# megvii-research/basedet

Measured on AMD Instinct MI355X. Metric: images/sec training RetinaNet-R50-FPN 1333x800, higher is better.
Workload: dtype bf16; 1 GPU; retinanet_r50_800x1344 train step (fwd+bwd+allreduce+SGD), DummyLoader boxes, random-init weights, inputs resident in HBM; per_gpu_batch=16, global_batch=16, parallelism=dp1

## Files before the change

### basedet_amd/csrc/gskip.hip

```cpp
#include "common.h"

namespace {

enum { GS_ANY = 1, GS_TOP = 2, GS_BOT = 4, GS_LEFT = 8, GS_RIGHT = 16, GS_TL = 32, GS_TR = 64, GS_BL = 128, GS_BR = 256 };

struct GsSeg { int patch_start, H, W, pw, off; };

struct GsParams {
    const bf16_raw* g;
    int* mask;
    int C, ppi, ph, pw_px, nseg, patches_per_img, total;
    GsSeg seg[BD_MAX_SEGS];
};

__device__ __forceinline__ int gs_level(const GsParams& p, int rem) {
    int s = 0;
#pragma unroll
    for (int k = 1; k < BD_MAX_SEGS; ++k)
        if (k < p.nseg && rem >= p.seg[k].patch_start) s = k;
    return s;
}

__global__ __launch_bounds__(256) void gskip_scan_kernel(const GsParams p) {
    __shared__ int sbits;
    const int tid = threadIdx.x;
    const int pid = blockIdx.x;
    const int n = pid / p.patches_per_img, rem = pid - n * p.patches_per_img;
    const int s = gs_level(p, rem);
    const int H = p.seg[s].H, W = p.seg[s].W, pwn = p.seg[s].pw;
    const int local = rem - p.seg[s].patch_start, by = local / pwn, bx = local - by * pwn;
    const int y0 = by * p.ph, x0 = bx * p.pw_px;
    const int cpp = p.C >> 3;
    const int items = p.ph * p.pw_px * cpp;
    const long long img = (long long)n * p.ppi + p.seg[s].off;
    if (tid == 0) sbits = 0;
    __syncthreads();
    int bits = 0;
    constexpr int U = 8;
    for (int b = 0; b < items; b += 256 * U) {
        u32x4_t v[U];
        int pix[U];
#pragma unroll
        for (int k = 0; k < U; ++k) {
            const int i = b + k * 256 + tid;
            v[k] = (u32x4_t){0u, 0u, 0u, 0u};
            pix[k] = -1;
            if (i < items) {
                const int px = i / cpp, ch = i - px * cpp;
                const int py = px / p.pw_px, pxx = px - py * p.pw_px;
                const int y = y0 + py, x = x0 + pxx;
                if (y < H && x < W) {
                    v[k] = *reinterpret_cast<const u32x4_t*>(p.g + (img + (long long)y * W + x) * p.C + ch * 8);
                    pix[k] = px;
                }
            }
        }
#pragma unroll
        for (int k = 0; k < U; ++k) {
            if (pix[k] >= 0 && (v[k][0] | v[k][1] | v[k][2] | v[k][3])) {
                const int py = pix[k] / p.pw_px, pxx = pix[k] - py * p.pw_px;
                const bool t = py == 0, bo = py == p.ph - 1, l = pxx == 0, r = pxx == p.pw_px - 1;
                bits |= GS_ANY | (t ? GS_TOP : 0) | (bo ? GS_BOT : 0) | (l ? GS_LEFT : 0) | (r ? GS_RIGHT : 0) | (t && l ? GS_TL : 0) |
                        (t && r ? GS_TR : 0) | (bo && l ? GS_BL : 0) | (bo && r ? GS_BR : 0);
            }
        }
    }
#pragma unroll
    for (int m = 32; m >= 1; m >>= 1) bits |= __shfl_xor(bits, m, 64);
    if ((tid & 63) == 0 && bits) atomicOr(&sbits, bits);
    __syncthreads();
    if (tid == 0) p.mask[pid] = sbits;
}

template <bool FRESH>
__device__ __forceinline__ int gs_mask(const int* m, int i) {
    if (FRESH) return __hip_atomic_load(m + i, __ATOMIC_RELAXED, __HIP_MEMORY_SCOPE_AGENT);
    return m[i];
}

template <bool FRESH>
__device__ __forceinline__ void gs_compact_body(const GsParams& p, int* live, int* list, int* count, int* wsum) {
    constexpr int KP = 8;
    const int tid = threadIdx.x, wv = tid >> 6, ln = tid & 63;
    int base = 0;
    for (int c0 = 0; c0 < p.total; c0 += 1024 * KP) {
        int lv[KP];
#pragma unroll
        for (int j = 0; j < KP; ++j) {
            const int q = c0 + tid * KP + j;
            lv[j] = 0;
            if (q < p.total) {
                const int n = q / p.patches_per_img, rem = q - n * p.patches_per_img;
                const int s = gs_level(p, rem);
                const int pwn = p.seg[s].pw, rows = (p.seg[s].H + p.ph - 1) / p.ph;
                const int local = rem - p.seg[s].patch_start, by = local / pwn, bx = local - by * pwn;
                const int* m = p.mask + (long long)n * p.patches_per_img + p.seg[s].patch_start;
                const bool up = by > 0, dn = by + 1 < rows, lf = bx > 0, rt = bx + 1 < pwn;
                int v = gs_mask<FRESH>(m, by * pwn + bx) & GS_ANY;
                if (up) v |= gs_mask<FRESH>(m, (by - 1) * pwn + bx) & GS_BOT;
                if (dn) v |= gs_mask<FRESH>(m, (by + 1) * pwn + bx) & GS_TOP;
                if (lf) v |= gs_mask<FRESH>(m, by * pwn + bx - 1) & GS_RIGHT;
                if (rt) v |= gs_mask<FRESH>(m, by * pwn + bx + 1) & GS_LEFT;
                if (up && lf) v |= gs_mask<FRESH>(m, (by - 1) * pwn + bx - 1) & GS_BR;
                if (up && rt) v |= gs_mask<FRESH>(m, (by - 1) * pwn + bx + 1) & GS_BL;
                if (dn && lf) v |= gs_mask<FRESH>(m, (by + 1) * pwn + bx - 1) & GS_TR;
                if (dn && rt) v |= gs_mask<FRESH>(m, (by + 1) * pwn + bx + 1) & GS_TL;
                lv[j] = v != 0;
            }
        }
        int cnt = 0;
#pragma unroll
        for (int j = 0; j < KP; ++j) cnt += lv[j];
        int inc = cnt;
#pragma unroll
        for (int o = 1; o < 64; o <<= 1) {
            const int y = __shfl_up(inc, o, 64);
            if (ln >= o) inc += y;
        }
        if (ln == 63) wsum[wv] = inc;
        __syncthreads();
        int off = base + inc - cnt, tot = 0;
#pragma unroll
        for (int w = 0; w < 16; ++w) {
            off += w < wv ? wsum[w] : 0;
            tot += wsum[w];
        }
#pragma unroll
        for (int j = 0; j < KP; ++j) {
            const int q = c0 + tid * KP + j;
            if (q < p.total) live[q] = lv[j];
            if (lv[j]) list[off++] = q;
        }
        base += tot;
        __syncthreads();
    }
    if (tid == 0) *count = base;
}

__global__ __launch_bounds__(1024) void gskip_compact_kernel(const GsParams p, int* live, int* list, int* count) {
    __shared__ int wsum[16];
    gs_compact_body<false>(p, live, list, count, wsum);
}

enum { GM_HDR = 8 };

struct GmSeg { int H, W, off, s4, s8, ss; };

struct GmParams {
    const bf16_raw* t;
    const int* live_in;
    int* map;
    int C, ppi, nseg, pi4, pi8, pis, tot4, tot8;
    GmSeg seg[BD_MAX_SEGS];
};

__global__ __launch_bounds__(1024) void gskip_fill_kernel(const GmParams p, const GsParams cp, int total) {
    __shared__ int sbits, slast;
    __shared__ int wsum[16];
    const int tid = threadIdx.x;
    int* m4 = p.map + GM_HDR;
    int* m8 = m4 + p.tot4;
    const int cpp = p.C >> 3;
    const int items = 4 * 16 * cpp;
    for (int pid = blockIdx.x; pid < total; pid += gridDim.x) {
        const int n = pid / p.pis, rem = pid - n * p.pis;
        int s = 0;
#pragma unroll
        for (int k = 1; k < BD_MAX_SEGS; ++k)
            if (k < p.nseg && rem >= p.seg[k].ss) s = k;
        const int H = p.seg[s].H, W = p.seg[s].W;
        const int sc = (W + 15) >> 4, r4 = (H + 3) >> 2, c8 = (W + 7) >> 3;
        const int local = rem - p.seg[s].ss, sy = local / sc, sx = local - sy * sc;
        int q4[2], q8[2];
        bool ok4[2], ok8[2], lv[2];
#pragma unroll
        for (int h = 0; h < 2; ++h) {
            ok4[h] = 2 * sy + h < r4;
            q4[h] = n * p.pi4 + p.seg[s].s4 + (2 * sy + h) * sc + sx;
            ok8[h] = 2 * sx + h < c8;
            q8[h] = n * p.pi8 + p.seg[s].s8 + sy * c8 + 2 * sx + h;
            lv[h] = ok4[h] && (p.live_in == nullptr || p.live_in[q4[h]] != 0);
        }
        int b = 0;
        if (lv[0] || lv[1]) {
            if (tid == 0) sbits = 0;
            __syncthreads();
            const long long img = (long long)n * p.ppi + p.seg[s].off;
            int bits = 0;
#pragma unroll
            for (int h = 0; h < 2; ++h) {
                if (!lv[h]) continue;
                for (int i = tid; i < items; i += 1024) {
                    const int px = i / cpp, ch = i - px * cpp;
                    const int py = px >> 4, pxx = px & 15;
                    const int y = 8 * sy + 4 * h + py, x = 16 * sx + pxx;
                    if (y < H && x < W) {
                        const u32x4_t v = *reinterpret_cast<const u32x4_t*>(p.t + (img + (long long)y * W + x) * p.C + ch * 8);
                        if (v[0] | v[1] | v[2] | v[3]) {
                            const bool t = py == 0, bo = py == 3, l = pxx == 0, r = pxx == 15;
                            const int w = GS_ANY | (t ? GS_TOP : 0) | (bo ? GS_BOT : 0) | (l ? GS_LEFT : 0) | (r ? GS_RIGHT : 0) |
                                          (t && l ? GS_TL : 0) | (t && r ? GS_TR : 0) | (bo && l ? GS_BL : 0) | (bo && r ? GS_BR : 0);
                            bits |= (w << (9 * h)) | (1 << (18 + (pxx >> 3)));
                        }
                    }
                }
            }
#pragma unroll
            for (int m = 32; m >= 1; m >>= 1) bits |= __shfl_xor(bits, m, 64);
            if ((tid & 63) == 0 && bits) atomicOr(&sbits, bits);
            __syncthreads();
            b = sbits;
            __syncthreads();
        }
        if (tid == 0) {
            if (ok4[0]) m4[q4[0]] = b & 511;
            if (ok4[1]) m4[q4[1]] = (b >> 9) & 511;
            if (ok8[0]) m8[q8[0]] = (b >> 18) & 1;
            if (ok8[1]) m8[q8[1]] = (b >> 19) & 1;
        }
    }
    if (tid == 0) {
        __builtin_amdgcn_fence(__ATOMIC_RELEASE, "agent");
        slast = atomicAdd(p.map + 1, 1) == (int)gridDim.x - 1;
    }
    __syncthreads();
    if (!slast) return;
    __builtin_amdgcn_fence(__ATOMIC_ACQUIRE, "agent");
    const int nxt = (p.map[0] & 1) ^ 1;
    int* live = m8 + p.tot8;
    gs_compact_body<true>(cp, live, live + p.tot4 * (1 + nxt), p.map + 2 + nxt, wsum);
    if (tid == 0) { p.map[0] = nxt; p.map[1] = 0; }
}

enum { FL_HDR = 8, FL_MAX_DEPTH = 8 };

struct FlSeg { int H, W, off, s4, pw; };

struct FlParams {
    const int* labels;
    int* map[FL_MAX_DEPTH];
    int A, ppi, nseg, depths, pi4, tot4;
    FlSeg seg[BD_MAX_SEGS];
};

__global__ __launch_bounds__(1024) void fwd_live_kernel(const FlParams p) {
    extern __shared__ __attribute__((aligned(16))) unsigned char fl_bm[];
    __shared__ int slast;
    __shared__ int wsum[16];
    const int tid = threadIdx.x;
    const int n = blockIdx.x / p.nseg, s = blockIdx.x - n * p.nseg;
    const int H = p.seg[s].H, W = p.seg[s].W, HW = H * W, pwn = p.seg[s].pw;
    const int npatch = ((H + 3) >> 2) * pwn;
    unsigned char* cur = fl_bm;
    unsigned char* nxt = fl_bm + HW;
    for (int i = tid; i < HW; i += 1024) cur[i] = 0;
    __syncthreads();
    const int* lab = p.labels + ((long long)n * p.ppi + p.seg[s].off) * p.A;
    for (int i = tid; i < HW * p.A; i += 1024)
        if (lab[i] > 0) cur[i / p.A] = 1;
    __syncthreads();
    for (int k = 0; k < p.depths; ++k) {
        for (int i = tid; i < HW; i += 1024) {
            const int y = i / W, x = i - y * W;
            const int y0 = y > 0 ? y - 1 : 0, y1 = y + 1 < H ? y + 1 : H - 1, x0 = x > 0 ? x - 1 : 0, x1 = x + 1 < W ? x + 1 : W - 1;
            int v = 0;
            for (int yy = y0; yy <= y1; ++yy)
                for (int xx = x0; xx <= x1; ++xx) v |= cur[yy * W + xx];
            nxt[i] = (unsigned char)v;
        }
        __syncthreads();
        int* live = p.map[k] + FL_HDR + n * p.pi4 + p.seg[s].s4;
        for (int q = tid; q < npatch; q += 1024) {
            const int by = q / pwn, bx = q - by * pwn;
            const int ye = by * 4 + 4 < H ? by * 4 + 4 : H, xe = bx * 16 + 16 < W ? bx * 16 + 16 : W;
            int v = 0;
            for (int y = by * 4; y < ye; ++y)
                for (int x = bx * 16; x < xe; ++x) v |= nxt[y * W + x];
            live[q] = v;
        }
        unsigned char* t = cur; cur = nxt; nxt = t;
        __syncthreads();
    }
    __builtin_amdgcn_fence(__ATOMIC_RELEASE, "agent");
    __syncthreads();
    if (tid == 0) slast = atomicAdd(p.map[0] + 1, 1) == (int)gridDim.x - 1;
    __syncthreads();
    if (!slast) return;
    __builtin_amdgcn_fence(__ATOMIC_ACQUIRE, "agent");
    constexpr int KP = 8;
    const int wv = tid >> 6, ln = tid & 63;
    for (int k = 0; k < p.depths; ++k) {
        int* hdr = p.map[k];
        const int* live = hdr + FL_HDR;
        const int to = (hdr[0] & 1) ^ 1;
        int* list = hdr + FL_HDR + p.tot4 * (1 + to);
        int base = 0;
        for (int c0 = 0; c0 < p.tot4; c0 += 1024 * KP) {
            int lv[KP];
            int cnt = 0;
#pragma unroll
            for (int j = 0; j < KP; ++j) {
                const int q = c0 + tid * KP + j;
                lv[j] = q < p.tot4 ? (__hip_atomic_load(live + q, __ATOMIC_RELAXED, __HIP_MEMORY_SCOPE_AGENT) != 0) : 0;
                cnt += lv[j];
            }
            int inc = cnt;
#pragma unroll
            for (int o = 1; o < 64; o <<= 1) {
                const int y = __shfl_up(inc, o, 64);
                if (ln >= o) inc += y;
            }
            if (ln == 63) wsum[wv] = inc;
            __syncthreads();
            int off = base + inc - cnt, tot = 0;
#pragma unroll
            for (int w = 0; w < 16; ++w) {
                off += w < wv ? wsum[w] : 0;
                tot += wsum[w];
            }
#pragma unroll
            for (int j = 0; j < KP; ++j)
                if (lv[j]) list[off++] = c0 + tid * KP + j;
            base += tot;
            __syncthreads();
        }
        if (tid == 0) { hdr[2 + to] = base; hdr[0] = to; }
    }
    if (tid == 0) p.map[0][1] = 0;
}

GsParams gs_params(const bd_conv_desc* d, int ph, int pw, int side = 0) {
    GsParams p{};
    p.C = side ? d->Cin : d->Cout; p.ppi = side ? d->in_pix_per_img : d->out_pix_per_img; p.ph = ph; p.pw_px = pw; p.nseg = d->nseg;
    int ps = 0;
    for (int s = 0; s < d->nseg; ++s) {
        GsSeg& sg = p.seg[s];
        const int H = side ? d->Hi[s] : d->Ho[s], W = side ? d->Wi[s] : d->Wo[s];
        sg.patch_start = ps; sg.H = H; sg.W = W; sg.pw = cdiv(W, pw); sg.off = side ? d->in_off[s] : d->out_off[s];
        ps += cdiv(H, ph) * sg.pw;
    }
    p.patches_per_img = ps;
    p.total = ps * d->N;
    return p;
}

}

int bd_gskip_patches(const bd_conv_desc* d, int ph, int pw) {
    return gs_params(d, ph, pw).total;
}

void bd_gskip_scan(const bd_conv_desc* d, const void* g, int ph, int pw, int* mask, hipStream_t stream) {
    GsParams p = gs_params(d, ph, pw);
    p.g = (const bf16_raw*)g; p.mask = mask;
    if (p.total > 0) hipLaunchKernelGGL(gskip_scan_kernel, dim3(p.total), dim3(256), 0, stream, p);
}

void bd_gskip_compact(const bd_conv_desc* d, int ph, int pw, const int* mask, int* live, int* list, int* count, hipStream_t stream) {
    GsParams p = gs_params(d, ph, pw);
    p.mask = const_cast<int*>(mask);
    hipLaunchKernelGGL(gskip_compact_kernel, dim3(1), dim3(1024), 0, stream, p, live, list, count);
}

void bd_gskip_map_layout(const bd_conv_desc* d, int side, BdGskipMap* out) {
    const int p4 = gs_params(d, 4, 16, side).total, p8 = gs_params(d, 8, 8, side).total;
    out->p4 = p4; out->p8 = p8;
    out->m4 = GM_HDR; out->m8 = GM_HDR + p4; out->live = out->m8 + p8; out->list = out->live + p4;
    out->ints = (size_t)GM_HDR + (size_t)4 * p4 + p8;
}

extern "C" size_t bd_conv2d_gskip_map_bytes(const bd_conv_desc* d, int of_dx) {
    if (!d || d->nseg < 1 || d->nseg > BD_MAX_SEGS || !(d->R == 3 && d->S == 3 && d->stride == 1 && d->pad == 1)) return 0;
    BdGskipMap m;
    bd_gskip_map_layout(d, of_dx ? 1 : 0, &m);
    return m.ints * sizeof(int);
}

void bd_gskip_fill(const bd_conv_desc* d, int side, const void* t, const int* live_in, int* map, hipStream_t stream) {
    const GsParams g4 = gs_params(d, 4, 16, side), g8 = gs_params(d, 8, 8, side), gs = gs_params(d, 8, 16, side);
    GmParams p{};
    p.t = (const bf16_raw*)t; p.live_in = live_in; p.map = map;
    p.C = g4.C; p.ppi = g4.ppi; p.nseg = g4.nseg;
    p.pi4 = g4.patches_per_img; p.pi8 = g8.patches_per_img; p.pis = gs.patches_per_img; p.tot4 = g4.total; p.tot8 = g8.total;
    for (int s = 0; s < g4.nseg; ++s)
        p.seg[s] = GmSeg{g4.seg[s].H, g4.seg[s].W, g4.seg[s].off, g4.seg[s].patch_start, g8.seg[s].patch_start, gs.seg[s].patch_start};
    GsParams cp = g4;
    cp.mask = map + GM_HDR;
    const int grid = gs.total < 128 ? gs.total : 128;
    if (grid > 0) hipLaunchKernelGGL(gskip_fill_kernel, dim3(grid), dim3(1024), 0, stream, p, cp, gs.total);
}

extern "C" int bd_gskip_map_scan(const bd_conv_desc* d, int of_dx, const void* t, void* map, size_t map_bytes, bd_stream_t stream) {
    BD_REQUIRE(d && t && map, "gskip_map_scan: null pointer");
    const size_t need = bd_conv2d_gskip_map_bytes(d, of_dx);
    BD_REQUIRE(need > 0, "gskip_map_scan: liveness maps belong to 3x3 / stride 1 / pad 1 descriptors");
    BD_REQUIRE(map_bytes >= need, "gskip_map_scan: map %zu < required %zu bytes", map_bytes, need);
    const int side = of_dx ? 1 : 0;
    BdGskipMap m;
    bd_gskip_map_layout(d, side, &m);
    int* mp = (int*)map;
    if (hipMemsetAsync(mp, 0, GM_HDR * sizeof(int), (hipStream_t)stream) != hipSuccess) { bd_set_error("gskip_map_scan: memset failed"); return BD_ELAUNCH; }
    GsParams p4 = gs_params(d, 4, 16, side), p8 = gs_params(d, 8, 8, side);
    p4.g = p8.g = (const bf16_raw*)t;
    p4.mask = mp + m.m4; p8.mask = mp + m.m8;
    if (p4.total > 0) {
        hipLaunchKernelGGL(gskip_scan_kernel, dim3(p4.total), dim3(256), 0, (hipStream_t)stream, p4);
        hipLaunchKernelGGL(gskip_scan_kernel, dim3(p8.total), dim3(256), 0, (hipStream_t)stream, p8);
    }
    hipLaunchKernelGGL(gskip_compact_kernel, dim3(1), dim3(1024), 0, (hipStream_t)stream, p4, mp + m.live, mp + m.list, mp + 2);
    BD_CHECK_LAUNCH("bd_gskip_map_scan");
    return BD_OK;
}

void bd_fwd_map_layout(const bd_conv_desc* d, BdFwdMap* out) {
    const int p4 = gs_params(d, 4, 16, 0).total;
    out->p4 = p4; out->live = FL_HDR; out->list = FL_HDR + p4;
    out->ints = (size_t)FL_HDR + (size_t)3 * p4;
}

extern "C" size_t bd_fwd_live_map_bytes(const bd_conv_desc* d) {
    if (!d || d->nseg < 1 || d->nseg > BD_MAX_SEGS || !(d->R == 3 && d->S == 3 && d->stride == 1 && d->pad == 1)) return 0;
    BdFwdMap m;
    bd_fwd_map_layout(d, &m);
    return m.ints * sizeof(int);
}

extern "C" int bd_fwd_live_maps(const bd_conv_desc* d, const int32_t* labels, int A, int depths, void* const* maps, size_t map_bytes,
                                int reset, bd_stream_t stream) {
    BD_REQUIRE(d && labels && maps, "fwd_live_maps: null pointer");
    const size_t need = bd_fwd_live_map_bytes(d);
    BD_REQUIRE(need > 0, "fwd_live_maps: forward liveness maps belong to 3x3 / stride 1 / pad 1 descriptors");
    BD_REQUIRE(A >= 1 && depths >= 1 && depths <= FL_MAX_DEPTH, "fwd_live_maps: A=%d depths=%d (1 .. %d)", A, depths, (int)FL_MAX_DEPTH);
    BD_REQUIRE(map_bytes >= need, "fwd_live_maps: map %zu < required %zu bytes", map_bytes, need);
    const GsParams g4 = gs_params(d, 4, 16, 0);
    FlParams p{};
    p.labels = labels; p.A = A; p.ppi = g4.ppi; p.nseg = g4.nseg; p.depths = depths; p.pi4 = g4.patches_per_img; p.tot4 = g4.total;
    size_t lds = 0;
    for (int s = 0; s < g4.nseg; ++s) {
        BD_REQUIRE(d->Hi[s] == d->Ho[s] && d->Wi[s] == d->Wo[s], "fwd_live_maps: level %d changes size", s);
        p.seg[s] = FlSeg{g4.seg[s].H, g4.seg[s].W, g4.seg[s].off, g4.seg[s].patch_start, g4.seg[s].pw};
        const size_t b = (size_t)2 * g4.seg[s].H * g4.seg[s].W;
        BD_REQUIRE((long long)g4.seg[s].H * g4.seg[s].W * A < 0x7fffffffll, "fwd_live_maps: level %d too large", s);
        lds = b > lds ? b : lds;
    }
    BD_REQUIRE(lds <= 160 * 1024 - 256, "fwd_live_maps: a level of %zu pixels does not fit the LDS bitmap", lds / 2);
    for (int k = 0; k < depths; ++k) {
        BD_REQUIRE(maps[k], "fwd_live_maps: null map %d", k);
        p.map[k] = (int*)maps[k];
        if (reset && hipMemsetAsync(maps[k], 0, FL_HDR * sizeof(int), (hipStream_t)stream) != hipSuccess) {
            bd_set_error("fwd_live_maps: memset failed");
            return BD_ELAUNCH;
        }
    }
    if (d->N < 1 || g4.total < 1) return BD_OK;
    BD_ONCE_PER_DEVICE((void)hipFuncSetAttribute(reinterpret_cast<const void*>(&fwd_live_kernel), hipFuncAttributeMaxDynamicSharedMemorySize,
                                                 160 * 1024 - 256));
    hipLaunchKernelGGL(fwd_live_kernel, dim3(d->N * g4.nseg), dim3(1024), lds, (hipStream_t)stream, p);
    BD_CHECK_LAUNCH("bd_fwd_live_maps");
    return BD_OK;
}
```

Baseline: 727.4 images/sec.

## Scan gradient-skip patches per wave and pack forward liveness into bitmaps

Adds a wave-per-patch scan kernel, used when patches are small, that covers four patches per wave and replaces integer division with a float-reciprocal division. The fill kernel now gives one fill patch to each wave instead of the whole 1024-thread block, gathers the mask writes in LDS and removes per-patch block barriers. The forward liveness kernel moves from a byte-per-pixel LDS map to a 32-pixel-per-word bitmap, with vectorised label loads and word-level 3x3 dilation. The aim is to cut launch, barrier and LDS costs in these auxiliary sparsity kernels, in exchange for more code paths and atomicOr contention while marking labels.

```diff
diff --git a/basedet_amd/csrc/gskip.hip b/basedet_amd/csrc/gskip.hip
--- a/basedet_amd/csrc/gskip.hip
+++ b/basedet_amd/csrc/gskip.hip
@@ -19,6 +19,25 @@
     for (int k = 1; k < BD_MAX_SEGS; ++k)
         if (k < p.nseg && rem >= p.seg[k].patch_start) s = k;
     return s;
+}
+
+__device__ __forceinline__ int gs_border_bits(int py, int pxx, int ph, int pw) {
+    const bool t = py == 0, bo = py == ph - 1, l = pxx == 0, r = pxx == pw - 1;
+    return GS_ANY | (t ? GS_TOP : 0) | (bo ? GS_BOT : 0) | (l ? GS_LEFT : 0) | (r ? GS_RIGHT : 0) | (t && l ? GS_TL : 0) |
+           (t && r ? GS_TR : 0) | (bo && l ? GS_BL : 0) | (bo && r ? GS_BR : 0);
+}
+
+__device__ __forceinline__ int gs_div(int i, int d, float inv) {
+    int q = (int)((float)i * inv);
+    q -= q * d > i;
+    q += (q + 1) * d <= i;
+    return q;
+}
+
+__device__ __forceinline__ int gs_wave_or(int bits) {
+#pragma unroll
+    for (int m = 32; m >= 1; m >>= 1) bits |= __shfl_xor(bits, m, 64);
+    return bits;
 }
 
 __global__ __launch_bounds__(256) void gskip_scan_kernel(const GsParams p) {
@@ -59,17 +78,64 @@
         for (int k = 0; k < U; ++k) {
             if (pix[k] >= 0 && (v[k][0] | v[k][1] | v[k][2] | v[k][3])) {
                 const int py = pix[k] / p.pw_px, pxx = pix[k] - py * p.pw_px;
-                const bool t = py == 0, bo = py == p.ph - 1, l = pxx == 0, r = pxx == p.pw_px - 1;
-                bits |= GS_ANY | (t ? GS_TOP : 0) | (bo ? GS_BOT : 0) | (l ? GS_LEFT : 0) | (r ? GS_RIGHT : 0) | (t && l ? GS_TL : 0) |
-                        (t && r ? GS_TR : 0) | (bo && l ? GS_BL : 0) | (bo && r ? GS_BR : 0);
-            }
-        }
-    }
-#pragma unroll
-    for (int m = 32; m >= 1; m >>= 1) bits |= __shfl_xor(bits, m, 64);
+                bits |= gs_border_bits(py, pxx, p.ph, p.pw_px);
+            }
+        }
+    }
+    bits = gs_wave_or(bits);
     if ((tid & 63) == 0 && bits) atomicOr(&sbits, bits);
     __syncthreads();
     if (tid == 0) p.mask[pid] = sbits;
+}
+
+enum { GS_WAVE_PATCHES = 4 };
+
+__global__ __launch_bounds__(256) void gskip_scan_wave_kernel(const GsParams p) {
+    const int ln = threadIdx.x & 63;
+    const int first = __builtin_amdgcn_readfirstlane((blockIdx.x * 4 + (threadIdx.x >> 6)) * GS_WAVE_PATCHES);
+    const int cpp = p.C >> 3;
+    const int items = p.ph * p.pw_px * cpp;
+    const float inv_cpp = 1.0f / (float)cpp, inv_pw = 1.0f / (float)p.pw_px;
+    constexpr int U = 8;
+    for (int j = 0; j < GS_WAVE_PATCHES; ++j) {
+        const int pid = first + j;
+        if (pid >= p.total) break;
+        const int n = pid / p.patches_per_img, rem = pid - n * p.patches_per_img;
+        const int s = gs_level(p, rem);
+        const int H = p.seg[s].H, W = p.seg[s].W, pwn = p.seg[s].pw;
+        const int local = rem - p.seg[s].patch_start, by = local / pwn, bx = local - by * pwn;
+        const int y0 = by * p.ph, x0 = bx * p.pw_px;
+        const long long img = (long long)n * p.ppi + p.seg[s].off;
+        int bits = 0;
+        for (int b = 0; b < items; b += 64 * U) {
+            u32x4_t v[U];
+            int pix[U];
+#pragma unroll
+            for (int k = 0; k < U; ++k) {
+                const int i = b + k * 64 + ln;
+                v[k] = (u32x4_t){0u, 0u, 0u, 0u};
+                pix[k] = -1;
+                if (i < items) {
+                    const int px = gs_div(i, cpp, inv_cpp), ch = i - px * cpp;
+                    const int py = gs_div(px, p.pw_px, inv_pw), pxx = px - py * p.pw_px;
+                    const int y = y0 + py, x = x0 + pxx;
+                    if (y < H && x < W) {
+                        v[k] = *reinterpret_cast<const u32x4_t*>(p.g + (img + (long long)y * W + x) * p.C + ch * 8);
+                        pix[k] = px;
+                    }
+                }
+            }
+#pragma unroll
+            for (int k = 0; k < U; ++k) {
+                if (pix[k] >= 0 && (v[k][0] | v[k][1] | v[k][2] | v[k][3])) {
+                    const int py = gs_div(pix[k], p.pw_px, inv_pw), pxx = pix[k] - py * p.pw_px;
+                    bits |= gs_border_bits(py, pxx, p.ph, p.pw_px);
+                }
+            }
+        }
+        bits = gs_wave_or(bits);
+        if (ln == 0) p.mask[pid] = bits;
+    }
 }
 
 template <bool FRESH>
@@ -142,7 +208,7 @@
     gs_compact_body<false>(p, live, list, count, wsum);
 }
 
-enum { GM_HDR = 8 };
+enum { GM_HDR = 8, GM_WAVES = 16 };
 
 struct GmSeg { int H, W, off, s4, s8, ss; };
 
@@ -155,76 +221,81 @@
 };
 
 __global__ __launch_bounds__(1024) void gskip_fill_kernel(const GmParams p, const GsParams cp, int total) {
-    __shared__ int sbits, slast;
+    __shared__ int slast;
+    __shared__ int sidx[GM_WAVES * 4], sval[GM_WAVES * 4];
     __shared__ int wsum[16];
-    const int tid = threadIdx.x;
+    const int tid = threadIdx.x, wv = tid >> 6, ln = tid & 63;
     int* m4 = p.map + GM_HDR;
-    int* m8 = m4 + p.tot4;
     const int cpp = p.C >> 3;
     const int items = 4 * 16 * cpp;
-    for (int pid = blockIdx.x; pid < total; pid += gridDim.x) {
-        const int n = pid / p.pis, rem = pid - n * p.pis;
-        int s = 0;
-#pragma unroll
-        for (int k = 1; k < BD_MAX_SEGS; ++k)
-            if (k < p.nseg && rem >= p.seg[k].ss) s = k;
-        const int H = p.seg[s].H, W = p.seg[s].W;
-        const int sc = (W + 15) >> 4, r4 = (H + 3) >> 2, c8 = (W + 7) >> 3;
-        const int local = rem - p.seg[s].ss, sy = local / sc, sx = local - sy * sc;
-        int q4[2], q8[2];
-        bool ok4[2], ok8[2], lv[2];
-#pragma unroll
-        for (int h = 0; h < 2; ++h) {
-            ok4[h] = 2 * sy + h < r4;
-            q4[h] = n * p.pi4 + p.seg[s].s4 + (2 * sy + h) * sc + sx;
-            ok8[h] = 2 * sx + h < c8;
-            q8[h] = n * p.pi8 + p.seg[s].s8 + sy * c8 + 2 * sx + h;
-            lv[h] = ok4[h] && (p.live_in == nullptr || p.live_in[q4[h]] != 0);
-        }
+    const float inv_cpp = 1.0f / (float)cpp;
+    constexpr int U = 8;
+    for (int base = blockIdx.x * GM_WAVES; base < total; base += gridDim.x * GM_WAVES) {
+        const int pid = __builtin_amdgcn_readfirstlane(base + wv);
+        int q4[2] = {-1, -1}, q8[2] = {-1, -1};
         int b = 0;
-        if (lv[0] || lv[1]) {
-            if (tid == 0) sbits = 0;
-            __syncthreads();
+        if (pid < total) {
+            const int n = pid / p.pis, rem = pid - n * p.pis;
+            int s = 0;
+#pragma unroll
+            for (int k = 1; k < BD_MAX_SEGS; ++k)
+                if (k < p.nseg && rem >= p.seg[k].ss) s = k;
+            const int H = p.seg[s].H, W = p.seg[s].W;
+            const int sc = (W + 15) >> 4, r4 = (H + 3) >> 2, c8 = (W + 7) >> 3;
+            const int local = rem - p.seg[s].ss, sy = local / sc, sx = local - sy * sc;
+            bool lv[2];
+#pragma unroll
+            for (int h = 0; h < 2; ++h) {
+                if (2 * sy + h < r4) q4[h] = n * p.pi4 + p.seg[s].s4 + (2 * sy + h) * sc + sx;
+                if (2 * sx + h < c8) q8[h] = p.tot4 + n * p.pi8 + p.seg[s].s8 + sy * c8 + 2 * sx + h;
+                lv[h] = q4[h] >= 0 && (p.live_in == nullptr || p.live_in[q4[h]] != 0);
+            }
             const long long img = (long long)n * p.ppi + p.seg[s].off;
-            int bits = 0;
 #pragma unroll
             for (int h = 0; h < 2; ++h) {
                 if (!lv[h]) continue;
-                for (int i = tid; i < items; i += 1024) {
-                    const int px = i / cpp, ch = i - px * cpp;
-                    const int py = px >> 4, pxx = px & 15;
-                    const int y = 8 * sy + 4 * h + py, x = 16 * sx + pxx;
-                    if (y < H && x < W) {
-                        const u32x4_t v = *reinterpret_cast<const u32x4_t*>(p.t + (img + (long long)y * W + x) * p.C + ch * 8);
-                        if (v[0] | v[1] | v[2] | v[3]) {
-                            const bool t = py == 0, bo = py == 3, l = pxx == 0, r = pxx == 15;
-                            const int w = GS_ANY | (t ? GS_TOP : 0) | (bo ? GS_BOT : 0) | (l ? GS_LEFT : 0) | (r ? GS_RIGHT : 0) |
-                                          (t && l ? GS_TL : 0) | (t && r ? GS_TR : 0) | (bo && l ? GS_BL : 0) | (bo && r ? GS_BR : 0);
-                            bits |= (w << (9 * h)) | (1 << (18 + (pxx >> 3)));
+                for (int i0 = 0; i0 < items; i0 += 64 * U) {
+                    u32x4_t v[U];
+                    int pix[U];
+#pragma unroll
+                    for (int k = 0; k < U; ++k) {
+                        const int i = i0 + k * 64 + ln;
+                        v[k] = (u32x4_t){0u, 0u, 0u, 0u};
+                        pix[k] = -1;
+                        if (i < items) {
+                            const int px = gs_div(i, cpp, inv_cpp), ch = i - px * cpp;
+                            const int y = 8 * sy + 4 * h + (px >> 4), x = 16 * sx + (px & 15);
+                            if (y < H && x < W) {
+                                v[k] = *reinterpret_cast<const u32x4_t*>(p.t + (img + (long long)y * W + x) * p.C + ch * 8);
+                                pix[k] = px;
+                            }
                         }
                     }
+#pragma unroll
+                    for (int k = 0; k < U; ++k)
+                        if (pix[k] >= 0 && (v[k][0] | v[k][1] | v[k][2] | v[k][3]))
+                            b |= (gs_border_bits(pix[k] >> 4, pix[k] & 15, 4, 16) << (9 * h)) | (1 << (18 + ((pix[k] & 15) >> 3)));
                 }
             }
-#pragma unroll
-            for (int m = 32; m >= 1; m >>= 1) bits |= __shfl_xor(bits, m, 64);
-            if ((tid & 63) == 0 && bits) atomicOr(&sbits, bits);
-            __syncthreads();
-            b = sbits;
-            __syncthreads();
-        }
-        if (tid == 0) {
-            if (ok4[0]) m4[q4[0]] = b & 511;
-            if (ok4[1]) m4[q4[1]] = (b >> 9) & 511;
-            if (ok8[0]) m8[q8[0]] = (b >> 18) & 1;
-            if (ok8[1]) m8[q8[1]] = (b >> 19) & 1;
-        }
-    }
-    if (tid == 0) {
+            if (lv[0] || lv[1]) b = gs_wave_or(b);
+        }
+        if (ln == 0) {
+            sidx[wv * 4 + 0] = q4[0]; sval[wv * 4 + 0] = b & 511;
+            sidx[wv * 4 + 1] = q4[1]; sval[wv * 4 + 1] = (b >> 9) & 511;
+            sidx[wv * 4 + 2] = q8[0]; sval[wv * 4 + 2] = (b >> 18) & 1;
+            sidx[wv * 4 + 3] = q8[1]; sval[wv * 4 + 3] = (b >> 19) & 1;
+        }
+        __syncthreads();
+        if (wv == 0 && sidx[ln] >= 0) m4[sidx[ln]] = sval[ln];
+        __syncthreads();
+    }
+    if (wv == 0) {
         __builtin_amdgcn_fence(__ATOMIC_RELEASE, "agent");
-        slast = atomicAdd(p.map + 1, 1) == (int)gridDim.x - 1;
+        if (ln == 0) slast = atomicAdd(p.map + 1, 1) == (int)gridDim.x - 1;
     }
     __syncthreads();
     if (!slast) return;
+    int* m8 = m4 + p.tot4;
     __builtin_amdgcn_fence(__ATOMIC_ACQUIRE, "agent");
     const int nxt = (p.map[0] & 1) ^ 1;
     int* live = m8 + p.tot8;
@@ -244,41 +315,70 @@
 };
 
 __global__ __launch_bounds__(1024) void fwd_live_kernel(const FlParams p) {
-    extern __shared__ __attribute__((aligned(16))) unsigned char fl_bm[];
+    extern __shared__ __attribute__((aligned(16))) unsigned fl_bm[];
     __shared__ int slast;
     __shared__ int wsum[16];
-    const int tid = threadIdx.x;
+    const int tid = threadIdx.x, wv = tid >> 6, ln = tid & 63;
     const int n = blockIdx.x / p.nseg, s = blockIdx.x - n * p.nseg;
-    const int H = p.seg[s].H, W = p.seg[s].W, HW = H * W, pwn = p.seg[s].pw;
-    const int npatch = ((H + 3) >> 2) * pwn;
-    unsigned char* cur = fl_bm;
-    unsigned char* nxt = fl_bm + HW;
-    for (int i = tid; i < HW; i += 1024) cur[i] = 0;
+    const int H = p.seg[s].H, W = p.seg[s].W, pwn = p.seg[s].pw;
+    const int wpr = (W + 31) >> 5, NW = H * wpr, prow = (H + 3) >> 2;
+    unsigned* cur = fl_bm;
+    unsigned* nxt = fl_bm + NW;
+    for (int i = tid; i < NW; i += 1024) cur[i] = 0;
     __syncthreads();
     const int* lab = p.labels + ((long long)n * p.ppi + p.seg[s].off) * p.A;
-    for (int i = tid; i < HW * p.A; i += 1024)
-        if (lab[i] > 0) cur[i / p.A] = 1;
+    const int total = H * W * p.A;
+    auto mark = [&](int e) {
+        const int px = e / p.A, y = px / W, x = px - y * W;
+        atomicOr(&cur[y * wpr + (x >> 5)], 1u << (x & 31));
+    };
+    int head = (int)((4 - ((reinterpret_cast<uintptr_t>(lab) >> 2) & 3)) & 3);
+    head = head < total ? head : total;
+    const int nvec = (total - head) >> 2, tail = head + 4 * nvec;
+    const u32x4_t* lab4 = reinterpret_cast<const u32x4_t*>(lab + head);
+    constexpr int FL_U = 8;
+    for (int v0 = 0; v0 < nvec; v0 += 1024 * FL_U) {
+        u32x4_t q[FL_U];
+#pragma unroll
+        for (int k = 0; k < FL_U; ++k) {
+            const int v = v0 + k * 1024 + tid;
+            q[k] = v < nvec ? lab4[v] : (u32x4_t){0u, 0u, 0u, 0u};
+        }
+#pragma unroll
+        for (int k = 0; k < FL_U; ++k) {
+            const int e = head + 4 * (v0 + k * 1024 + tid);
+#pragma unroll
+            for (int c = 0; c < 4; ++c)
+                if ((int)q[k][c] > 0) mark(e + c);
+        }
+    }
+    if (tid < head && lab[tid] > 0) mark(tid);
+    if (tid < total - tail && lab[tail + tid] > 0) mark(tail + tid);
     __syncthreads();
     for (int k = 0; k < p.depths; ++k) {
-        for (int i = tid; i < HW; i += 1024) {
-            const int y = i / W, x = i - y * W;
-            const int y0 = y > 0 ? y - 1 : 0, y1 = y + 1 < H ? y + 1 : H - 1, x0 = x > 0 ? x - 1 : 0, x1 = x + 1 < W ? x + 1 : W - 1;
-            int v = 0;
-            for (int yy = y0; yy <= y1; ++yy)
-                for (int xx = x0; xx <= x1; ++xx) v |= cur[yy * W + xx];
-            nxt[i] = (unsigned char)v;
+        for (int i = tid; i < NW; i += 1024) {
+            const int y = i / wpr, j = i - y * wpr;
+            const unsigned rowmask = (j == wpr - 1 && (W & 31)) ? (1u << (W & 31)) - 1u : 0xffffffffu;
+            const int y0 = y > 0 ? y - 1 : 0, y1 = y + 1 < H ? y + 1 : H - 1;
+            unsigned acc = 0;
+            for (int yy = y0; yy <= y1; ++yy) {
+                const unsigned* r = cur + yy * wpr;
+                const unsigned c = r[j], lw = j > 0 ? r[j - 1] : 0u, rw = j + 1 < wpr ? r[j + 1] : 0u;
+                acc |= c | (c << 1) | (c >> 1) | (lw >> 31) | (rw << 31);
+            }
+            nxt[i] = acc & rowmask;
         }
         __syncthreads();
         int* live = p.map[k] + FL_HDR + n * p.pi4 + p.seg[s].s4;
-        for (int q = tid; q < npatch; q += 1024) {
-            const int by = q / pwn, bx = q - by * pwn;
-            const int ye = by * 4 + 4 < H ? by * 4 + 4 : H, xe = bx * 16 + 16 < W ? bx * 16 + 16 : W;
-            int v = 0;
-            for (int y = by * 4; y < ye; ++y)
-                for (int x = bx * 16; x < xe; ++x) v |= nxt[y * W + x];
-            live[q] = v;
-        }
-        unsigned char* t = cur; cur = nxt; nxt = t;
+        for (int by = wv; by < prow; by += 16) {
+            const int ye = by * 4 + 4 < H ? by * 4 + 4 : H;
+            for (int bx = ln; bx < pwn; bx += 64) {
+                unsigned v = 0;
+                for (int y = by * 4; y < ye; ++y) v |= nxt[y * wpr + (bx >> 1)];
+                live[by * pwn + bx] = ((v >> (16 * (bx & 1))) & 0xffffu) != 0;
+            }
+        }
+        unsigned* t = cur; cur = nxt; nxt = t;
         __syncthreads();
     }
     __builtin_amdgcn_fence(__ATOMIC_RELEASE, "agent");
@@ -288,7 +388,6 @@
     if (!slast) return;
     __builtin_amdgcn_fence(__ATOMIC_ACQUIRE, "agent");
     constexpr int KP = 8;
-    const int wv = tid >> 6, ln = tid & 63;
     for (int k = 0; k < p.depths; ++k) {
         int* hdr = p.map[k];
         const int* live = hdr + FL_HDR;
@@ -344,6 +443,14 @@
     return p;
 }
 
+void gs_launch_scan(const GsParams& p, hipStream_t stream) {
+    if (p.total < 1) return;
+    if ((long long)p.C * 2 * p.ph * p.pw_px < 256 * 8 * 16)
+        hipLaunchKernelGGL(gskip_scan_wave_kernel, dim3(cdiv(p.total, 4 * GS_WAVE_PATCHES)), dim3(256), 0, stream, p);
+    else
+        hipLaunchKernelGGL(gskip_scan_kernel, dim3(p.total), dim3(256), 0, stream, p);
+}
+
 }
 
 int bd_gskip_patches(const bd_conv_desc* d, int ph, int pw) {
@@ -353,7 +460,7 @@
 void bd_gskip_scan(const bd_conv_desc* d, const void* g, int ph, int pw, int* mask, hipStream_t stream) {
     GsParams p = gs_params(d, ph, pw);
     p.g = (const bf16_raw*)g; p.mask = mask;
-    if (p.total > 0) hipLaunchKernelGGL(gskip_scan_kernel, dim3(p.total), dim3(256), 0, stream, p);
+    gs_launch_scan(p, stream);
 }
 
 void bd_gskip_compact(const bd_conv_desc* d, int ph, int pw, const int* mask, int* live, int* list, int* count, hipStream_t stream) {
@@ -386,7 +493,9 @@
         p.seg[s] = GmSeg{g4.seg[s].H, g4.seg[s].W, g4.seg[s].off, g4.seg[s].patch_start, g8.seg[s].patch_start, gs.seg[s].patch_start};
     GsParams cp = g4;
     cp.mask = map + GM_HDR;
-    const int grid = gs.total < 128 ? gs.total : 128;
+    static_assert(GM_WAVES * 64 == 1024 && GM_WAVES * 4 == 64, "gskip_fill_kernel: one wave per block, wave 0 stores the visit's words");
+    const int wgs = cdiv(gs.total, GM_WAVES);
+    const int grid = wgs < 256 ? wgs : 256;
     if (grid > 0) hipLaunchKernelGGL(gskip_fill_kernel, dim3(grid), dim3(1024), 0, stream, p, cp, gs.total);
 }
 
@@ -403,10 +512,8 @@
     GsParams p4 = gs_params(d, 4, 16, side), p8 = gs_params(d, 8, 8, side);
     p4.g = p8.g = (const bf16_raw*)t;
     p4.mask = mp + m.m4; p8.mask = mp + m.m8;
-    if (p4.total > 0) {
-        hipLaunchKernelGGL(gskip_scan_kernel, dim3(p4.total), dim3(256), 0, (hipStream_t)stream, p4);
-        hipLaunchKernelGGL(gskip_scan_kernel, dim3(p8.total), dim3(256), 0, (hipStream_t)stream, p8);
-    }
+    gs_launch_scan(p4, (hipStream_t)stream);
+    gs_launch_scan(p8, (hipStream_t)stream);
     hipLaunchKernelGGL(gskip_compact_kernel, dim3(1), dim3(1024), 0, (hipStream_t)stream, p4, mp + m.live, mp + m.list, mp + 2);
     BD_CHECK_LAUNCH("bd_gskip_map_scan");
     return BD_OK;
@@ -439,11 +546,11 @@
     for (int s = 0; s < g4.nseg; ++s) {
         BD_REQUIRE(d->Hi[s] == d->Ho[s] && d->Wi[s] == d->Wo[s], "fwd_live_maps: level %d changes size", s);
         p.seg[s] = FlSeg{g4.seg[s].H, g4.seg[s].W, g4.seg[s].off, g4.seg[s].patch_start, g4.seg[s].pw};
-        const size_t b = (size_t)2 * g4.seg[s].H * g4.seg[s].W;
+        const size_t b = (size_t)2 * g4.seg[s].H * cdiv(g4.seg[s].W, 32) * sizeof(unsigned);
         BD_REQUIRE((long long)g4.seg[s].H * g4.seg[s].W * A < 0x7fffffffll, "fwd_live_maps: level %d too large", s);
         lds = b > lds ? b : lds;
     }
-    BD_REQUIRE(lds <= 160 * 1024 - 256, "fwd_live_maps: a level of %zu pixels does not fit the LDS bitmap", lds / 2);
+    BD_REQUIRE(lds <= 160 * 1024 - 256, "fwd_live_maps: a level's bitmaps (%zu bytes) do not fit the LDS", lds);
     for (int k = 0; k < depths; ++k) {
         BD_REQUIRE(maps[k], "fwd_live_maps: null map %d", k);
         p.map[k] = (int*)maps[k];
```

Result: no change. 732.8 images/sec, median of 6 (+0.7%).
